# CVPR23/Depth-guided-Texture-Diffusion-for-Image-Semantic-Segmentation

Measured on AMD Instinct MI355X. Metric: training images/sec (512x512 RGB-D, bs=8 per GPU; fwd+loss+bwd+allreduce+AdamW), higher is better.
Workload: dtype bf16; 1 GPU; config/sod.yml model `cod` (pvt_v2_b2 + ConvNeXt-B texture diffuser + Hitnet decoder), 512x512 RGB+depth, batch 8/GPU, random init, DropPath active; mode=train, global_batch=8, parallelism=dp1, hip_graph=True, graph_mode=single

## Files before the change

depth-guided-texture-diffusion-for-image-semantic-segmentation_amd/csrc/attn_bwd.hip:

```cpp
#include "common.h"

namespace {

constexpr float LOG2E = 1.4426950408889634f;
constexpr int SLICE = 256;

template <typename T>
__global__ __launch_bounds__(256) void attn_delta_kernel(const T* __restrict__ o, const T* __restrict__ dout,
                                                         float* __restrict__ delta, int B, int N, int heads) {
  typedef typename Vec16<T>::type VT;
  constexpr int V = Vec16<T>::N, LPR = 64 / V;
  const int64_t total = (int64_t)B * N * heads;
  const int64_t gid = ((int64_t)blockIdx.x * 256 + threadIdx.x);
  const int64_t item = gid / LPR;
  const int sub = (int)(gid % LPR);
  float s = 0.f;
  int64_t bn = 0; int hd = 0;
  if (item < total) {
    bn = item / heads; hd = (int)(item % heads);
    const size_t off = ((size_t)bn * heads + hd) * 64 + sub * V;
    VT a = *reinterpret_cast<const VT*>(o + off);
    VT g = *reinterpret_cast<const VT*>(dout + off);
#pragma unroll
    for (int j = 0; j < V; ++j) s += (float)a[j] * (float)g[j];
  }
  s = group_sum(s, LPR);
  if (item < total && sub == 0) {
    const int64_t b = bn / N, n = bn % N;
    delta[((size_t)b * heads + hd) * N + n] = s;
  }
}

template <typename T>
struct DkdvSmem {
  static constexpr int QS = 72;
  T q[2][32][QS];
  T g[2][32][QS];
  float lse2[2][32];
  float dl[2][32];
};

constexpr int KGROUP = 128;
constexpr int64_t DKDV_MAX_WGS = 1024;
constexpr int64_t DKDV_SLAB_BYTES = DKDV_MAX_WGS * 65536;

template <typename T>
__global__ __launch_bounds__(256, 2) void sra_bwd_dkdv_bf16(const T* __restrict__ q, const T* __restrict__ kv,
                                                            const T* __restrict__ dout, const float* __restrict__ lse,
                                                            const float* __restrict__ delta, float* __restrict__ dkv,
                                                            int N, int Nkv, int heads, int kgroups, float scale, int qch,
                                                            int64_t slab_stride) {
  typedef T bf16_t;
  typedef typename Vec16<T>::type bf16x8;
  __shared__ __attribute__((aligned(16))) DkdvSmem<T> sm;
  constexpr int QS = DkdvSmem<T>::QS;
  const int C = heads * 64;
  const int b = blockIdx.z, hd = blockIdx.y / kgroups, kg = blockIdx.y % kgroups;
  const int tid = threadIdx.x, wave = tid >> 6, lane = tid & 63, r = lane & 31, h = lane >> 5;
  const float sl2 = scale * LOG2E;
  const bf16_t* kvb = kv + (size_t)b * Nkv * 2 * C + hd * 64;
  const size_t sbase = ((size_t)b * heads + hd) * N;
  const int qt_begin = blockIdx.x * qch;
  const int qt_end = min(qt_begin + qch, (N + 31) / 32);
  const int ktile0 = kg * KGROUP + wave * 32;
  const bool wave_active = ktile0 < Nkv;
  const int key = ktile0 + r;
  const bool kok = key < Nkv;

  auto stage_load = [&](int q0, bf16x8 (&v)[2], float& sv) {
#pragma unroll
    for (int k = 0; k < 2; ++k) {
      const int row = tid >> 3, ch = tid & 7;
      if (q0 + row < N) v[k] = *reinterpret_cast<const bf16x8*>((k ? dout : q) + ((size_t)b * N + q0 + row) * C + hd * 64 + ch * 8);
      else
#pragma unroll
        for (int j = 0; j < 8; ++j) v[k][j] = (bf16_t)0.f;
    }
    if (tid < 64) {
      const int row = tid & 31;
      const bool ok = (q0 + row) < N;
      sv = tid < 32 ? (ok ? lse[sbase + q0 + row] * LOG2E : INFINITY) : (ok ? delta[sbase + q0 + row] : 0.f);
    }
  };
  auto stage_store = [&](int buf, const bf16x8 (&v)[2], float sv) {
    const int row = tid >> 3, ch = tid & 7;
    *reinterpret_cast<bf16x8*>(&sm.q[buf][row][ch * 8]) = v[0];
    *reinterpret_cast<bf16x8*>(&sm.g[buf][row][ch * 8]) = v[1];
    if (tid < 32) sm.lse2[buf][tid] = sv;
    else if (tid < 64) sm.dl[buf][tid - 32] = sv;
  };

  bf16x8 kf[4], vf[4];
  {
    const bf16_t* kp = kvb + (size_t)key * 2 * C + 8 * h;
#pragma unroll
    for (int s = 0; s < 4; ++s) {
      if (kok) { kf[s] = *reinterpret_cast<const bf16x8*>(kp + 16 * s); vf[s] = *reinterpret_cast<const bf16x8*>(kp + C + 16 * s); }
      else
#pragma unroll
        for (int j = 0; j < 8; ++j) { kf[s][j] = (bf16_t)0.f; vf[s][j] = (bf16_t)0.f; }
    }
  }
  f32x16 dk[2], dv[2];
#pragma unroll
  for (int i = 0; i < 16; ++i) { dk[0][i] = dk[1][i] = dv[0][i] = dv[1][i] = 0.f; }

  bf16x8 st[2];
  float sv = 0.f;
  stage_load(qt_begin * 32, st, sv);
  stage_store(0, st, sv);
  __syncthreads();
  int cur = 0;
#pragma unroll 1
  for (int qt = qt_begin; qt < qt_end; ++qt) {
    const bool more = (qt + 1) < qt_end;
    if (more) stage_load((qt + 1) * 32, st, sv);
    if (wave_active) {
      f32x16 sA, pA;
#pragma unroll
      for (int i = 0; i < 16; ++i) { sA[i] = 0.f; pA[i] = 0.f; }
#pragma unroll
      for (int s = 0; s < 4; ++s) {
        const bf16x8 qf = *reinterpret_cast<const bf16x8*>(&sm.q[cur][r][16 * s + 8 * h]);
        const bf16x8 gf = *reinterpret_cast<const bf16x8*>(&sm.g[cur][r][16 * s + 8 * h]);
        sA = mfma16(qf, kf[s], sA);
        pA = mfma16(gf, vf[s], pA);
      }
#pragma unroll
      for (int i = 0; i < 16; ++i) {
        const int qi = mfma_row(i, h);
        const float p = kok ? __builtin_amdgcn_exp2f(fmaf(sA[i], sl2, -sm.lse2[cur][qi])) : 0.f;
        sA[i] = p;
        pA[i] = p * (pA[i] - sm.dl[cur][qi]) * scale;
      }
#pragma unroll
      for (int s2 = 0; s2 < 2; ++s2) {
        bf16x8 pf, df;
#pragma unroll
        for (int j = 0; j < 8; ++j) { pf[j] = (bf16_t)sA[8 * s2 + j]; df[j] = (bf16_t)pA[8 * s2 + j]; }
#pragma unroll
        for (int nb = 0; nb < 2; ++nb) {
          const bf16x8 gb = lds_tr_frag(&sm.g[cur][0][0], QS, 16 * s2, nb * 32, lane);
          const bf16x8 qb = lds_tr_frag(&sm.q[cur][0][0], QS, 16 * s2, nb * 32, lane);
          dv[nb] = mfma16(pf, gb, dv[nb]);
          dk[nb] = mfma16(df, qb, dk[nb]);
        }
      }
    }
    if (more) stage_store(cur ^ 1, st, sv);
    __syncthreads();
    cur ^= 1;
  }
  if (wave_active) {
#pragma unroll
    for (int nb = 0; nb < 2; ++nb)
#pragma unroll
      for (int i = 0; i < 16; ++i) {
        const int kk = ktile0 + mfma_row(i, h);
        if (kk < Nkv) {
          float* p = dkv + (size_t)blockIdx.x * slab_stride + ((size_t)b * Nkv + kk) * 2 * C + hd * 64 + nb * 32 + r;
          p[0] = dk[nb][i];
          p[C] = dv[nb][i];
        }
      }
  }
}

__global__ __launch_bounds__(256) void dkdv_reduce_kernel(const float* __restrict__ slab, float* __restrict__ dkv, int64_t n4, int chunks,
                                                          int64_t stride4) {
  const f32x4* s4 = reinterpret_cast<const f32x4*>(slab);
  f32x4* o4 = reinterpret_cast<f32x4*>(dkv);
  for (int64_t i = (int64_t)blockIdx.x * 256 + threadIdx.x; i < n4; i += (int64_t)gridDim.x * 256) {
    f32x4 acc = s4[i];
    for (int c = 1; c < chunks; ++c) {
      const f32x4 v = s4[i + (int64_t)c * stride4];
      acc[0] += v[0]; acc[1] += v[1]; acc[2] += v[2]; acc[3] += v[3];
    }
    o4[i] = acc;
  }
// ... 364 lines not shown
```

depth-guided-texture-diffusion-for-image-semantic-segmentation_amd/csrc/common.h:

```cpp
#pragma once
#include <hip/hip_runtime.h>
#include <stdint.h>
#include <stdio.h>
#include <stdlib.h>
#include "../../include/dgtd.h"

typedef __bf16 bf16_t;
typedef __bf16 bf16x8 __attribute__((ext_vector_type(8)));
typedef __bf16 bf16x4 __attribute__((ext_vector_type(4)));
typedef _Float16 f16_t;
typedef _Float16 f16x8 __attribute__((ext_vector_type(8)));
typedef _Float16 f16x4 __attribute__((ext_vector_type(4)));
typedef float f32x4 __attribute__((ext_vector_type(4)));
typedef float f32x16 __attribute__((ext_vector_type(16)));

void dgtd_set_error(const char* fmt, ...);
#define DGTD_FAIL(code, ...) do { dgtd_set_error(__VA_ARGS__); return (code); } while (0)
#define DGTD_REQUIRE(cond, ...) do { if (!(cond)) DGTD_FAIL(2, __VA_ARGS__); } while (0)
#define DGTD_CHECK_LAUNCH(name) do { hipError_t e_ = hipGetLastError(); \
    if (e_ != hipSuccess) DGTD_FAIL(3, "%s: launch failed: %s", name, hipGetErrorString(e_)); } while (0)

struct DgtdProfScope {
  bool on;
  hipEvent_t a, b;
  hipStream_t st;
  int bound;
  double amount;
  char key[112];
  DgtdProfScope(hipStream_t st, int bound, double amount, const char* fmt, ...) __attribute__((format(printf, 5, 6)));
  ~DgtdProfScope();
};
#define DGTD_PROF(st, bound, amount, ...) DgtdProfScope dgtd_prof_scope_((hipStream_t)(st), (bound), (double)(amount), __VA_ARGS__)
enum { DGTD_HBM = 0, DGTD_MFMA = 1 };
static inline int dgtd_esize(dgtd_dtype dt) { return (dt == DGTD_BF16 || dt == DGTD_F16) ? 2 : (dt == DGTD_F64 ? 8 : 4); }

template <typename T> __device__ __forceinline__ float to_f(T v) { return (float)v; }
template <typename T> __device__ __forceinline__ T from_f(float v) { return (T)v; }

template <typename T> struct Vec16;
template <> struct Vec16<float> { static constexpr int N = 4; typedef f32x4 type; };
template <> struct Vec16<bf16_t> { static constexpr int N = 8; typedef bf16x8 type; };
template <> struct Vec16<f16_t> { static constexpr int N = 8; typedef f16x8 type; };
template <typename T> struct Vec8;
template <> struct Vec8<bf16_t> { typedef bf16x4 type; };
template <> struct Vec8<f16_t> { typedef f16x4 type; };
template <typename T> struct Vec2;
template <> struct Vec2<float> { typedef float type __attribute__((ext_vector_type(2))); };
template <> struct Vec2<bf16_t> { typedef bf16_t type __attribute__((ext_vector_type(2))); };
template <> struct Vec2<f16_t> { typedef f16_t type __attribute__((ext_vector_type(2))); };

__device__ __forceinline__ f32x16 mfma16(bf16x8 a, bf16x8 b, f32x16 c) { return __builtin_amdgcn_mfma_f32_32x32x16_bf16(a, b, c, 0, 0, 0); }
__device__ __forceinline__ f32x16 mfma16(f16x8 a, f16x8 b, f32x16 c) { return __builtin_amdgcn_mfma_f32_32x32x16_f16(a, b, c, 0, 0, 0); }

#define DGTD_IS_HALF(dt) ((dt) == DGTD_BF16 || (dt) == DGTD_F16)
#define DGTD_DISPATCH(dt, STMT) do { if ((dt) == DGTD_BF16) { typedef bf16_t T_; STMT; } else if ((dt) == DGTD_F16) { typedef f16_t T_; STMT; } \
                                     else { typedef float T_; STMT; } } while (0)
#define DGTD_DISPATCH_HALF(dt, STMT) do { if ((dt) == DGTD_F16) { typedef f16_t T_; STMT; } else { typedef bf16_t T_; STMT; } } while (0)
#define DGTD_DISPATCH_K37(K, STMT) do { if ((K) == 7) { constexpr int K_ = 7; STMT; } else { constexpr int K_ = 3; STMT; } } while (0)

static inline long env_int(const char* name, long dflt) { const char* e = getenv(name); return e ? atol(e) : dflt; }

__device__ __forceinline__ float wave_sum(float v) {
#pragma unroll
  for (int o = 32; o > 0; o >>= 1) v += __shfl_xor(v, o, 64);
  return v;
}
__device__ __forceinline__ float wave_max(float v) {
#pragma unroll
  for (int o = 32; o > 0; o >>= 1) v = fmaxf(v, __shfl_xor(v, o, 64));
  return v;
}
__device__ __forceinline__ float group_sum(float v, int g) {
  for (int o = g >> 1; o > 0; o >>= 1) v += __shfl_xor(v, o, 64);
  return v;
}

__device__ __forceinline__ constexpr int mfma_row(int reg, int h) { return (reg & 3) + 8 * (reg >> 2) + 4 * h; }

typedef short s16x4 __attribute__((ext_vector_type(4)));
template <typename T>
__device__ __forceinline__ typename Vec16<T>::type lds_tr_frag(const T* base, int stride, int row0, int col0, int lane) {
  const int i = lane & 15, g1 = (lane >> 4) & 1, h = lane >> 5;
  const T* p = base + (row0 + 4 * h + (i >> 2)) * stride + col0 + 16 * g1 + 4 * (i & 3);
  typedef s16x4 __attribute__((address_space(3))) * lds_ptr;
  typedef typename Vec8<T>::type V4;
  s16x4 lo = __builtin_amdgcn_ds_read_tr16_b64_v4i16((lds_ptr)p);
  s16x4 hi = __builtin_amdgcn_ds_read_tr16_b64_v4i16((lds_ptr)(p + 8 * stride));
  V4 l4 = __builtin_bit_cast(V4, lo), h4 = __builtin_bit_cast(V4, hi);
  typename Vec16<T>::type f;
#pragma unroll
  for (int j = 0; j < 4; ++j) { f[j] = l4[j]; f[4 + j] = h4[j]; }
  return f;
}

__device__ __forceinline__ float gelu_phi(float x, float* pdf) {
  const float a = fabsf(x) * 0.70710678118654752f;
  const float t = __builtin_amdgcn_rcpf(fmaf(0.3275911f, a, 1.f));
  const float q = t * fmaf(t, fmaf(t, fmaf(t, fmaf(t, 1.061405429f, -1.453152027f), 1.421413741f), -0.284496736f), 0.254829592f);
  const float e = __builtin_amdgcn_exp2f(-a * a * 1.4426950408889634f);
  const float hc = 0.5f * q * e;
  *pdf = 0.3989422804014327f * e;
  return x >= 0.f ? 1.f - hc : hc;
}
__device__ __forceinline__ float gelu_fast(float x) { float pdf; return x * gelu_phi(x, &pdf); }
__device__ __forceinline__ float gelu_grad_fast(float x) { float pdf; const float phi = gelu_phi(x, &pdf); return fmaf(x, pdf, phi); }

static inline int64_t cdiv(int64_t a, int64_t b) { return (a + b - 1) / b; }

int dgtd_multi_reduce_impl(const dgtd_reduce_entry* entries, int n, hipStream_t st);
```

depth-guided-texture-diffusion-for-image-semantic-segmentation_amd/csrc/dwconv_tiled.hip:

```cpp
#include "common.h"

namespace {

constexpr int TY = 4, TXW = 16, TXS = 8;

template <typename T, int K>
__device__ __forceinline__ void stage_tile(T* __restrict__ tile, const T* __restrict__ x, int b, int y0, int x0, int cb, int H, int W,
                                           int C, int tid) {
  typedef typename Vec16<T>::type VT;
  constexpr int V = Vec16<T>::N, P = K / 2, RW = TXW + K - 1, RH = TY + K - 1, CPP = 128 / V;
  constexpr int TOTAL = RH * RW * CPP, NCH = (TOTAL + 255) / 256;
  VT v[NCH];
#pragma unroll
  for (int k = 0; k < NCH; ++k) {
    const int i = tid + k * 256;
    const int ch = i % CPP, pos = i / CPP, xx = pos % RW, yy = pos / RW;
    const int gy = y0 + yy - P, gx = x0 + xx - P;
    if (i < TOTAL && gy >= 0 && gy < H && gx >= 0 && gx < W) v[k] = *reinterpret_cast<const VT*>(x + (((size_t)b * H + gy) * W + gx) * C + cb * 128 + ch * V);
    else
#pragma unroll
      for (int j = 0; j < V; ++j) v[k][j] = (T)0.f;
  }
#pragma unroll
  for (int k = 0; k < NCH; ++k) {
    const int i = tid + k * 256;
    if (i < TOTAL) *reinterpret_cast<VT*>(tile + (size_t)i * V) = v[k];
  }
}

template <typename T, int K, int MODE>
__global__ __launch_bounds__(256) void dwconv_tiled_fwd_kernel(const T* __restrict__ x, const float* __restrict__ wt,
                                                               const float* __restrict__ bias, const T* __restrict__ aux,
                                                               T* __restrict__ y, int B, int H, int W, int C) {
  typedef typename Vec2<T>::type PT;
  constexpr int P = K / 2, RW = TXW + K - 1;
  extern __shared__ __attribute__((aligned(16))) char smem[];
  T* tile = reinterpret_cast<T*>(smem);
  const int tid = threadIdx.x, lane = tid & 63, wave = tid >> 6;
  const int ncb = C / 128, txn = (W + TXW - 1) / TXW, tyn = (H + TY - 1) / TY;
  const int nb = gridDim.x, xcd = blockIdx.x & 7, qn = nb >> 3, rn = nb & 7;
  int t = (xcd < rn ? xcd * (qn + 1) : rn * (qn + 1) + (xcd - rn) * qn) + (blockIdx.x >> 3);
  const int cb = t % ncb; t /= ncb;
  const int ty = t % tyn; t /= tyn;
  const int tx = t % txn;
  const int b = t / txn;
  const int y0 = ty * TY, x0 = tx * TXW, c0 = cb * 128 + lane * 2;
  stage_tile<T, K>(tile, x, b, y0, x0, cb, H, W, C, tid);
  typedef float f2 __attribute__((ext_vector_type(2)));
  f2 w[K * K];
#pragma unroll
  for (int i = 0; i < K * K; ++i) { w[i][0] = wt[(size_t)i * C + c0]; w[i][1] = wt[(size_t)i * C + c0 + 1]; }
  f2 bv;
  bv[0] = bias ? bias[c0] : 0.f; bv[1] = bias ? bias[c0 + 1] : 0.f;
  __syncthreads();
  const int oy = y0 + wave;
  if (oy >= H) return;
#pragma unroll 1
  for (int s = 0; s < TXW / TXS; ++s) {
    const int sx = s * TXS;
    if (x0 + sx >= W) break;
    f2 acc[TXS];
#pragma unroll
    for (int i = 0; i < TXS; ++i) acc[i] = bv;
#pragma unroll
    for (int ky = 0; ky < K; ++ky) {
      f2 in[TXS + K - 1];
      const T* row = tile + ((size_t)(wave + ky) * RW + sx) * 128 + lane * 2;
#pragma unroll
      for (int i = 0; i < TXS + K - 1; ++i) {
        PT v = *reinterpret_cast<const PT*>(row + (size_t)i * 128);
        in[i][0] = (float)v[0]; in[i][1] = (float)v[1];
      }
#pragma unroll
      for (int kx = 0; kx < K; ++kx)
#pragma unroll
        for (int i = 0; i < TXS; ++i) acc[i] = __builtin_elementwise_fma(in[i + kx], w[ky * K + kx], acc[i]);
    }
#pragma unroll
    for (int i = 0; i < TXS; ++i) {
      const int ox = x0 + sx + i;
      if (ox < W) {
        const size_t o = (((size_t)b * H + oy) * W + ox) * C + c0;
        PT r;
        if (MODE == 2) {
          PT g = *reinterpret_cast<const PT*>(aux + o);
          r[0] = (T)((float)g[0] * gelu_grad_fast(acc[i][0])); r[1] = (T)((float)g[1] * gelu_grad_fast(acc[i][1]));
        } else if (MODE == 1) {
          r[0] = (T)gelu_fast(acc[i][0]); r[1] = (T)gelu_fast(acc[i][1]);
        } else if (MODE == 3) {
          PT g = *reinterpret_cast<const PT*>(aux + o);
          r[0] = (T)(acc[i][0] + (float)g[0]); r[1] = (T)(acc[i][1] + (float)g[1]);
        } else {
          r[0] = (T)acc[i][0]; r[1] = (T)acc[i][1];
        }
        *reinterpret_cast<PT*>(y + o) = r;
      }
    }
  }
}

template <typename T, int K> constexpr size_t fwd_lds() { return (size_t)(TY + K - 1) * (TXW + K - 1) * 128 * sizeof(T); }

}

template <typename T, int K>
static int tiled_fwd(const void* x, const float* wt, const float* bias, const void* aux, void* y, int B, int H, int W, int C, int mode,
                     hipStream_t s) {
  const int64_t tiles = (int64_t)B * cdiv(H, TY) * cdiv(W, TXW) * (C / 128);
  DGTD_REQUIRE(tiles < (1LL << 31), "dwconv_tiled_fwd: too many tiles");
  const size_t lds = fwd_lds<T, K>();
#define TILED(MODE) hipLaunchKernelGGL((dwconv_tiled_fwd_kernel<T, K, MODE>), dim3((unsigned)tiles), dim3(256), lds, s, (const T*)x, wt, bias, (const T*)aux, (T*)y, B, H, W, C)
  if (mode == 0) TILED(0); else if (mode == 1) TILED(1); else if (mode == 2) TILED(2); else TILED(3);
#undef TILED
  DGTD_CHECK_LAUNCH("dwconv_tiled_fwd");
  return 0;
}

int dgtd_dwconv_tiled_fwd(const void* x, const float* wt, const float* bias, const void* aux, void* y, int B, int H, int W, int C, int K,
                          int mode, dgtd_dtype dt, hipStream_t s) {
  DGTD_REQUIRE(K == 7, "dwconv_tiled_fwd: K=%d (the tiled kernel serves 7x7 only)", K);
  DGTD_DISPATCH(dt, return (tiled_fwd<T_, 7>(x, wt, bias, aux, y, B, H, W, C, mode, s)));
}
```

depth-guided-texture-diffusion-for-image-semantic-segmentation_amd/csrc/layernorm.hip:

```cpp
#include "common.h"

namespace {

constexpr int LN_MAX_NPL = 4;
constexpr int LN_BWD_MAX_GRID = 1024;

template <typename T>
struct RowRegs {
  static constexpr int V = Vec16<T>::N;
  float v[LN_MAX_NPL][V];
};

template <typename T, int NPL>
__device__ __forceinline__ void load_row(const T* __restrict__ p, int cpr, int gl, int G, float (&v)[NPL][Vec16<T>::N]) {
  typedef typename Vec16<T>::type VT;
  constexpr int V = Vec16<T>::N;
#pragma unroll
  for (int i = 0; i < NPL; ++i) {
    int c = gl + i * G;
    if (c < cpr) {
      VT t = *reinterpret_cast<const VT*>(p + (size_t)c * V);
#pragma unroll
      for (int j = 0; j < V; ++j) v[i][j] = (float)t[j];
    } else {
#pragma unroll
      for (int j = 0; j < V; ++j) v[i][j] = 0.f;
    }
  }
}

template <typename T, int NPL>
__global__ __launch_bounds__(256) void ln_fwd_kernel(const T* __restrict__ x, const float* __restrict__ gamma,
                                                     const float* __restrict__ beta, T* __restrict__ y,
                                                     float* __restrict__ mean, float* __restrict__ rstd,
                                                     int64_t rows, int C, float eps, int G) {
  typedef typename Vec16<T>::type VT;
  constexpr int V = Vec16<T>::N;
  const int cpr = C / V;
  const int lane = threadIdx.x & 63, wave = threadIdx.x >> 6;
  const int gl = lane & (G - 1), gi = lane / G, rpw = 64 / G;
  const int64_t rows_per_block = (int64_t)rpw * 4;
  const float invC = 1.f / (float)C;
  float gm[NPL][V], bt[NPL][V];
#pragma unroll
  for (int i = 0; i < NPL; ++i) {
    int c = gl + i * G;
#pragma unroll
    for (int j = 0; j < V; ++j) {
      gm[i][j] = (c < cpr) ? gamma[c * V + j] : 0.f;
      bt[i][j] = (c < cpr) ? beta[c * V + j] : 0.f;
    }
  }
  constexpr int U = (NPL <= 2) ? 4 : 2;
  for (int64_t r0 = (int64_t)blockIdx.x * rows_per_block * U; r0 < rows; r0 += (int64_t)gridDim.x * rows_per_block * U) {
    float v[U][NPL][V];
    bool ok[U];
#pragma unroll
    for (int u = 0; u < U; ++u) {
      const int64_t row = r0 + (int64_t)u * rows_per_block + wave * rpw + gi;
      ok[u] = row < rows;
      if (ok[u]) load_row<T, NPL>(x + row * C, cpr, gl, G, v[u]);
      else {
#pragma unroll
        for (int i = 0; i < NPL; ++i)
#pragma unroll
          for (int j = 0; j < V; ++j) v[u][i][j] = 0.f;
      }
    }
#pragma unroll
    for (int u = 0; u < U; ++u) {
      const int64_t row = r0 + (int64_t)u * rows_per_block + wave * rpw + gi;
      float s = 0.f;
#pragma unroll
      for (int i = 0; i < NPL; ++i)
#pragma unroll
        for (int j = 0; j < V; ++j) s += v[u][i][j];
      const float mu = group_sum(s, G) * invC;
      float q = 0.f;
#pragma unroll
      for (int i = 0; i < NPL; ++i) {
        bool in = (gl + i * G) < cpr;
#pragma unroll
        for (int j = 0; j < V; ++j) { float d = in ? v[u][i][j] - mu : 0.f; q += d * d; }
      }
      const float rs = rsqrtf(group_sum(q, G) * invC + eps);
      if (ok[u]) {
#pragma unroll
        for (int i = 0; i < NPL; ++i) {
          int c = gl + i * G;
          if (c < cpr) {
            VT o;
#pragma unroll
            for (int j = 0; j < V; ++j) o[j] = (T)((v[u][i][j] - mu) * rs * gm[i][j] + bt[i][j]);
            *reinterpret_cast<VT*>(y + row * C + (size_t)c * V) = o;
          }
        }
        if (gl == 0) { mean[row] = mu; rstd[row] = rs; }
      }
    }
  }
}

template <typename T, int NPL>
__global__ __launch_bounds__(256) void ln_bwd_kernel(const T* __restrict__ dy, const T* __restrict__ x,
                                                     const float* __restrict__ gamma, const float* __restrict__ mean,
                                                     const float* __restrict__ rstd, const T* __restrict__ dres, T* __restrict__ dx,
                                                     float* __restrict__ ws, int64_t rows, int C, int G) {
  typedef typename Vec16<T>::type VT;
  constexpr int V = Vec16<T>::N;
  extern __shared__ float red[];
  const int cpr = C / V;
  const int lane = threadIdx.x & 63, wave = threadIdx.x >> 6;
  const int gl = lane & (G - 1), gi = lane / G, rpw = 64 / G;
  const int64_t rows_per_block = (int64_t)rpw * 4;
  const float invC = 1.f / (float)C;
  float gm[NPL][V], dg[NPL][V], db[NPL][V];
#pragma unroll
  for (int i = 0; i < NPL; ++i) {
    int c = gl + i * G;
#pragma unroll
    for (int j = 0; j < V; ++j) { gm[i][j] = (c < cpr) ? gamma[c * V + j] : 0.f; dg[i][j] = 0.f; db[i][j] = 0.f; }
  }
  constexpr int U = (NPL <= 2) ? 4 : 2;
  for (int64_t r0 = (int64_t)blockIdx.x * rows_per_block * U; r0 < rows; r0 += (int64_t)gridDim.x * rows_per_block * U) {
    float xv[U][NPL][V], gv[U][NPL][V], mu[U], rs[U];
    bool ok[U];
#pragma unroll
    for (int u = 0; u < U; ++u) {
      const int64_t row = r0 + (int64_t)u * rows_per_block + wave * rpw + gi;
      ok[u] = row < rows;
      if (ok[u]) {
        load_row<T, NPL>(x + row * C, cpr, gl, G, xv[u]);
        load_row<T, NPL>(dy + row * C, cpr, gl, G, gv[u]);
        mu[u] = mean[row]; rs[u] = rstd[row];
      } else {
        mu[u] = 0.f; rs[u] = 0.f;
#pragma unroll
        for (int i = 0; i < NPL; ++i)
#pragma unroll
          for (int j = 0; j < V; ++j) { xv[u][i][j] = 0.f; gv[u][i][j] = 0.f; }
      }
    }
#pragma unroll
    for (int u = 0; u < U; ++u) {
      float a = 0.f, b = 0.f;
#pragma unroll
      for (int i = 0; i < NPL; ++i) {
        bool in = (gl + i * G) < cpr;
#pragma unroll
        for (int j = 0; j < V; ++j) {
          float xh = in ? (xv[u][i][j] - mu[u]) * rs[u] : 0.f;
          float g = gv[u][i][j];
          dg[i][j] += g * xh;
          db[i][j] += g;
          g *= gm[i][j];
          a += g; b += g * xh;
          xv[u][i][j] = xh; gv[u][i][j] = g;
        }
      }
      a = group_sum(a, G) * invC;
      b = group_sum(b, G) * invC;
      if (ok[u]) {
        const int64_t row = r0 + (int64_t)u * rows_per_block + wave * rpw + gi;
#pragma unroll
        for (int i = 0; i < NPL; ++i) {
          int c = gl + i * G;
          if (c < cpr) {
            VT o, r;
            if (dres) r = *reinterpret_cast<const VT*>(dres + row * C + (size_t)c * V);
#pragma unroll
            for (int j = 0; j < V; ++j) o[j] = (T)(rs[u] * (gv[u][i][j] - a - xv[u][i][j] * b) + (dres ? (float)r[j] : 0.f));
            *reinterpret_cast<VT*>(dx + row * C + (size_t)c * V) = o;
          }
        }
      }
    }
  }
#pragma unroll
  for (int i = 0; i < NPL; ++i)
#pragma unroll
    for (int j = 0; j < V; ++j)
      for (int o = G; o < 64; o <<= 1) { dg[i][j] += __shfl_xor(dg[i][j], o, 64); db[i][j] += __shfl_xor(db[i][j], o, 64); }
  if (gi == 0) {
#pragma unroll
    for (int i = 0; i < NPL; ++i) {
      int c = gl + i * G;
      if (c < cpr)
#pragma unroll
        for (int j = 0; j < V; ++j) { red[(wave * 2 + 0) * C + c * V + j] = dg[i][j]; red[(wave * 2 + 1) * C + c * V + j] = db[i][j]; }
    }
  }
  __syncthreads();
  for (int c = threadIdx.x; c < 2 * C; c += 256) {
    int which = c / C, col = c % C;
    float s = 0.f;
#pragma unroll
    for (int w = 0; w < 4; ++w) s += red[(w * 2 + which) * C + col];
    ws[((size_t)blockIdx.x * 2 + which) * C + col] = s;
  }
}

struct LnGeom { int G, npl; int64_t rows_per_block; };
template <typename T> LnGeom ln_geom(int C) {
  int cpr = C / Vec16<T>::N;
  int G = 1;
  while (G < cpr && G < 64) G <<= 1;
  LnGeom g; g.G = G; g.npl = (cpr + G - 1) / G; g.rows_per_block = (64 / G) * 4;
  return g;
}

template <typename T>
int ln_fwd_launch(const void* x, const float* gamma, const float* beta, void* y, float* mean, float* rstd,
                  int64_t rows, int C, float eps, hipStream_t s) {
  DGTD_REQUIRE(C % Vec16<T>::N == 0, "layernorm: C=%d must be a multiple of %d", C, Vec16<T>::N);
  LnGeom g = ln_geom<T>(C);
  DGTD_REQUIRE(g.npl <= LN_MAX_NPL, "layernorm: C=%d too large", C);
  if (rows == 0) return 0;
  const int U = g.npl <= 2 ? 4 : 2;
  int grid = (int)std::min<int64_t>(cdiv(rows, g.rows_per_block * U), 256 * 8);
#define LN_FWD(NPL) hipLaunchKernelGGL((ln_fwd_kernel<T, NPL>), dim3(grid), dim3(256), 0, s, (const T*)x, gamma, beta, (T*)y, mean, rstd, rows, C, eps, g.G)
  switch (g.npl) { case 1: LN_FWD(1); break; case 2: LN_FWD(2); break; case 3: LN_FWD(3); break; default: LN_FWD(4); }
#undef LN_FWD
  DGTD_CHECK_LAUNCH("layernorm_fwd");
  return 0;
}

template <typename T>
int ln_bwd_launch(const void* dy, const void* x, const float* gamma, const float* mean, const float* rstd, void* dx,
                  float* dgamma, float* dbeta, void* ws, int64_t rows, int C, hipStream_t s, const void* dres = nullptr, int* nblocks = nullptr) {
  DGTD_REQUIRE(C % Vec16<T>::N == 0, "layernorm: C=%d must be a multiple of %d", C, Vec16<T>::N);
  LnGeom g = ln_geom<T>(C);
  DGTD_REQUIRE(g.npl <= LN_MAX_NPL, "layernorm: C=%d too large", C);
  DGTD_REQUIRE(rows > 0, "layernorm_bwd: rows must be > 0");
  int grid = (int)std::min<int64_t>(cdiv(rows, g.rows_per_block * 4), LN_BWD_MAX_GRID);
  size_t lds = (size_t)4 * 2 * C * sizeof(float);
#define LN_BWD(NPL) hipLaunchKernelGGL((ln_bwd_kernel<T, NPL>), dim3(grid), dim3(256), lds, s, (const T*)dy, (const T*)x, gamma, mean, rstd, (const T*)dres, (T*)dx, (float*)ws, rows, C, g.G)
  switch (g.npl) { case 1: LN_BWD(1); break; case 2: LN_BWD(2); break; case 3: LN_BWD(3); break; default: LN_BWD(4); }
#undef LN_BWD
  DGTD_CHECK_LAUNCH("layernorm_bwd");
  if (nblocks) { *nblocks = grid; return 0; }
  const dgtd_reduce_entry e{(const float*)ws, grid, 2 * C, dgamma, C, dbeta, DGTD_F32, 0, 0, nullptr};
  return dgtd_multi_reduce_impl(&e, 1, s);
}

}

extern "C" int dgtd_layernorm_fwd(const void* x, const float* gamma, const float* beta, void* y, float* mean, float* rstd,
                                  int64_t rows, int C, float eps, dgtd_dtype dt, dgtd_stream s) {
  DGTD_PROF(s, DGTD_HBM, 2.0 * dgtd_esize(dt) * rows * C, "dgtd_layernorm_fwd[rows=%lld,C=%d]", (long long)rows, C);
  DGTD_REQUIRE(DGTD_IS_HALF(dt) || dt == DGTD_F32, "layernorm_fwd: bad dtype %d", (int)dt);
  DGTD_DISPATCH(dt, return ln_fwd_launch<T_>(x, gamma, beta, y, mean, rstd, rows, C, eps, (hipStream_t)s));
}

extern "C" int dgtd_layernorm_bwd_add(const void* dy, const void* x, const float* gamma, const float* mean, const float* rstd,
                                      const void* dx_add, void* dx, float* dgamma, float* dbeta, void* workspace, int64_t rows, int C,
                                      dgtd_dtype dt, dgtd_stream s) {
  DGTD_PROF(s, DGTD_HBM, (dx_add ? 4.0 : 3.0) * dgtd_esize(dt) * rows * C, "dgtd_layernorm_bwd[rows=%lld,C=%d]", (long long)rows, C);
  DGTD_REQUIRE(DGTD_IS_HALF(dt) || dt == DGTD_F32, "layernorm_bwd_add: bad dtype %d", (int)dt);
  DGTD_DISPATCH(dt, return ln_bwd_launch<T_>(dy, x, gamma, mean, rstd, dx, dgamma, dbeta, workspace, rows, C, (hipStream_t)s, dx_add));
}

extern "C" int dgtd_layernorm_bwd_partial(const void* dy, const void* x, const float* gamma, const float* mean, const float* rstd,
                                          const void* dx_add, void* dx, void* workspace, int64_t rows, int C, dgtd_dtype dt, int* nblocks,
                                          dgtd_stream s) {
  DGTD_REQUIRE(nblocks, "layernorm_bwd_partial: nblocks is NULL");
  DGTD_PROF(s, DGTD_HBM, (dx_add ? 4.0 : 3.0) * dgtd_esize(dt) * rows * C, "dgtd_layernorm_bwd[rows=%lld,C=%d]", (long long)rows, C);
  DGTD_REQUIRE(DGTD_IS_HALF(dt) || dt == DGTD_F32, "layernorm_bwd_partial: bad dtype %d", (int)dt);
  DGTD_DISPATCH(dt, return ln_bwd_launch<T_>(dy, x, gamma, mean, rstd, dx, nullptr, nullptr, workspace, rows, C, (hipStream_t)s, dx_add, nblocks));
}

extern "C" int64_t dgtd_layernorm_bwd_workspace(int C) { return (int64_t)LN_BWD_MAX_GRID * 2 * C * sizeof(float); }

extern "C" int dgtd_layernorm_bwd(const void* dy, const void* x, const float* gamma, const float* mean, const float* rstd,
                                  void* dx, float* dgamma, float* dbeta, void* workspace, int64_t rows, int C,
                                  dgtd_dtype dt, dgtd_stream s) {
  DGTD_PROF(s, DGTD_HBM, 3.0 * dgtd_esize(dt) * rows * C, "dgtd_layernorm_bwd[rows=%lld,C=%d]", (long long)rows, C);
  DGTD_REQUIRE(DGTD_IS_HALF(dt) || dt == DGTD_F32, "layernorm_bwd: bad dtype %d", (int)dt);
  DGTD_DISPATCH(dt, return ln_bwd_launch<T_>(dy, x, gamma, mean, rstd, dx, dgamma, dbeta, workspace, rows, C, (hipStream_t)s));
}
```

Measured before the change: 275.5 images/s.

## Use DPP/permlane reductions, compile-time LN group size, and prefetch in dwconv

Replaces shuffle-based warp reductions with DPP and permlane swap intrinsics and makes the group size a template parameter. LayerNorm forward and backward now batch the group reductions across rows, clamp row indices so loads are unconditional, and are dispatched per (NPL, G). The depthwise conv tile stage splits its loads from its LDS stores, with clamped addresses instead of branches, and prefetches the aux (gradient or residual) inputs before the barrier. The aim is less cross-lane shuffle latency and better memory-level parallelism, at the cost of more template instantiations and more registers in use.

```diff
diff --git a/depth-guided-texture-diffusion-for-image-semantic-segmentation_amd/csrc/attn_bwd.hip b/depth-guided-texture-diffusion-for-image-semantic-segmentation_amd/csrc/attn_bwd.hip
--- a/depth-guided-texture-diffusion-for-image-semantic-segmentation_amd/csrc/attn_bwd.hip
+++ b/depth-guided-texture-diffusion-for-image-semantic-segmentation_amd/csrc/attn_bwd.hip
@@ -24,7 +24,7 @@
 #pragma unroll
     for (int j = 0; j < V; ++j) s += (float)a[j] * (float)g[j];
   }
-  s = group_sum(s, LPR);
+  s = group_sum<LPR>(s);
   if (item < total && sub == 0) {
     const int64_t b = bn / N, n = bn % N;
     delta[((size_t)b * heads + hd) * N + n] = s;
diff --git a/depth-guided-texture-diffusion-for-image-semantic-segmentation_amd/csrc/common.h b/depth-guided-texture-diffusion-for-image-semantic-segmentation_amd/csrc/common.h
--- a/depth-guided-texture-diffusion-for-image-semantic-segmentation_amd/csrc/common.h
+++ b/depth-guided-texture-diffusion-for-image-semantic-segmentation_amd/csrc/common.h
@@ -60,20 +60,51 @@
 
 static inline long env_int(const char* name, long dflt) { const char* e = getenv(name); return e ? atol(e) : dflt; }
 
-__device__ __forceinline__ float wave_sum(float v) {
+struct LaneAdd { __device__ __forceinline__ float operator()(float a, float b) const { return a + b; } };
+struct LaneMax { __device__ __forceinline__ float operator()(float a, float b) const { return fmaxf(a, b); } };
+
+template <int CTRL, int BANK_MASK>
+__device__ __forceinline__ float dpp_move(float old, float v) {
+  return __builtin_bit_cast(float, __builtin_amdgcn_update_dpp(__builtin_bit_cast(int, old), __builtin_bit_cast(int, v), CTRL, 0xF, BANK_MASK, false));
+}
+template <int O, bool INV8 = false, typename Op>
+__device__ __forceinline__ float lane_xor_combine(float v, Op op) {
+  static_assert(O == 1 || O == 2 || O == 4 || O == 8 || O == 16 || O == 32, "lane_xor_combine: O must be a power of two below 64");
+  if constexpr (O == 1) return op(v, dpp_move<0xB1, 0xF>(v, v));
+  else if constexpr (O == 2) return op(v, dpp_move<0x4E, 0xF>(v, v));
+  else if constexpr (O == 4 && INV8) return op(v, dpp_move<0x124, 0xF>(v, v));
+  else if constexpr (O == 4) return op(v, dpp_move<0x114, 0xA>(dpp_move<0x104, 0x5>(v, v), v));
+  else if constexpr (O == 8) return op(v, dpp_move<0x128, 0xF>(v, v));
+  else {
+    const unsigned u = __builtin_bit_cast(unsigned, v);
+    const auto r = (O == 16) ? __builtin_amdgcn_permlane16_swap(u, u, false, false) : __builtin_amdgcn_permlane32_swap(u, u, false, false);
+    return op(__builtin_bit_cast(float, (unsigned)r[0]), __builtin_bit_cast(float, (unsigned)r[1]));
+  }
+}
+template <int G, int N, typename Op>
+__device__ __forceinline__ void group_reduce(float (&v)[N], Op op) {
+  static_assert(G == 1 || G == 2 || G == 4 || G == 8 || G == 16 || G == 32 || G == 64, "group_reduce: G must be a power of two <= 64");
 #pragma unroll
-  for (int o = 32; o > 0; o >>= 1) v += __shfl_xor(v, o, 64);
-  return v;
+  for (int n = 0; n < N; ++n) if constexpr (G >= 64) v[n] = lane_xor_combine<32>(v[n], op);
+#pragma unroll
+  for (int n = 0; n < N; ++n) if constexpr (G >= 32) v[n] = lane_xor_combine<16>(v[n], op);
+#pragma unroll
+  for (int n = 0; n < N; ++n) if constexpr (G >= 16) v[n] = lane_xor_combine<8>(v[n], op);
+#pragma unroll
+  for (int n = 0; n < N; ++n) if constexpr (G >= 8) v[n] = lane_xor_combine<4, (G >= 16)>(v[n], op);
+#pragma unroll
+  for (int n = 0; n < N; ++n) if constexpr (G >= 4) v[n] = lane_xor_combine<2>(v[n], op);
+#pragma unroll
+  for (int n = 0; n < N; ++n) if constexpr (G >= 2) v[n] = lane_xor_combine<1>(v[n], op);
 }
-__device__ __forceinline__ float wave_max(float v) {
+template <int O, int N> __device__ __forceinline__ void lane_xor_add(float (&v)[N]) {
 #pragma unroll
-  for (int o = 32; o > 0; o >>= 1) v = fmaxf(v, __shfl_xor(v, o, 64));
-  return v;
+  for (int n = 0; n < N; ++n) v[n] = lane_xor_combine<O>(v[n], LaneAdd());
 }
-__device__ __forceinline__ float group_sum(float v, int g) {
-  for (int o = g >> 1; o > 0; o >>= 1) v += __shfl_xor(v, o, 64);
-  return v;
-}
+template <int G, int N> __device__ __forceinline__ void group_sum(float (&v)[N]) { group_reduce<G>(v, LaneAdd()); }
+template <int G> __device__ __forceinline__ float group_sum(float v) { float a[1] = {v}; group_reduce<G>(a, LaneAdd()); return a[0]; }
+__device__ __forceinline__ float wave_sum(float v) { return group_sum<64>(v); }
+__device__ __forceinline__ float wave_max(float v) { float a[1] = {v}; group_reduce<64>(a, LaneMax()); return a[0]; }
 
 __device__ __forceinline__ constexpr int mfma_row(int reg, int h) { return (reg & 3) + 8 * (reg >> 2) + 4 * h; }
 
diff --git a/depth-guided-texture-diffusion-for-image-semantic-segmentation_amd/csrc/dwconv_tiled.hip b/depth-guided-texture-diffusion-for-image-semantic-segmentation_amd/csrc/dwconv_tiled.hip
--- a/depth-guided-texture-diffusion-for-image-semantic-segmentation_amd/csrc/dwconv_tiled.hip
+++ b/depth-guided-texture-diffusion-for-image-semantic-segmentation_amd/csrc/dwconv_tiled.hip
@@ -5,27 +5,40 @@
 constexpr int TY = 4, TXW = 16, TXS = 8;
 
 template <typename T, int K>
-__device__ __forceinline__ void stage_tile(T* __restrict__ tile, const T* __restrict__ x, int b, int y0, int x0, int cb, int H, int W,
-                                           int C, int tid) {
+struct TileStage {
   typedef typename Vec16<T>::type VT;
-  constexpr int V = Vec16<T>::N, P = K / 2, RW = TXW + K - 1, RH = TY + K - 1, CPP = 128 / V;
-  constexpr int TOTAL = RH * RW * CPP, NCH = (TOTAL + 255) / 256;
+  static constexpr int V = Vec16<T>::N, P = K / 2, RW = TXW + K - 1, RH = TY + K - 1, CPP = 128 / V;
+  static constexpr int TOTAL = RH * RW * CPP, NCH = (TOTAL + 255) / 256, SLOTS = NCH * 256;
   VT v[NCH];
+  bool ok[NCH];
+  __device__ __forceinline__ void load(const T* __restrict__ x, int b, int y0, int x0, int cb, int H, int W, int C, int tid) {
 #pragma unroll
-  for (int k = 0; k < NCH; ++k) {
-    const int i = tid + k * 256;
-    const int ch = i % CPP, pos = i / CPP, xx = pos % RW, yy = pos / RW;
-    const int gy = y0 + yy - P, gx = x0 + xx - P;
-    if (i < TOTAL && gy >= 0 && gy < H && gx >= 0 && gx < W) v[k] = *reinterpret_cast<const VT*>(x + (((size_t)b * H + gy) * W + gx) * C + cb * 128 + ch * V);
-    else
+    for (int k = 0; k < NCH; ++k) {
+      const int i = tid + k * 256;
+      const int ch = i % CPP, pos = i / CPP, xx = pos % RW, yy = pos / RW;
+      const int gy = y0 + yy - P, gx = x0 + xx - P;
+      ok[k] = i < TOTAL && gy >= 0 && gy < H && gx >= 0 && gx < W;
+      const int cy = min(max(gy, 0), H - 1), cx = min(max(gx, 0), W - 1);
+      v[k] = *reinterpret_cast<const VT*>(x + (((size_t)b * H + cy) * W + cx) * C + cb * 128 + ch * V);
+    }
+  }
+  __device__ __forceinline__ void store(T* __restrict__ tile, int tid) const {
 #pragma unroll
-      for (int j = 0; j < V; ++j) v[k][j] = (T)0.f;
+    for (int k = 0; k < NCH; ++k) {
+      const int i = tid + k * 256;
+      VT o;
+#pragma unroll
+      for (int j = 0; j < V; ++j) o[j] = ok[k] ? v[k][j] : (T)0.f;
+      *reinterpret_cast<VT*>(tile + (size_t)i * V) = o;
+    }
   }
-#pragma unroll
-  for (int k = 0; k < NCH; ++k) {
-    const int i = tid + k * 256;
-    if (i < TOTAL) *reinterpret_cast<VT*>(tile + (size_t)i * V) = v[k];
-  }
+};
+
+template <typename P>
+__device__ __forceinline__ void pin_here(P& v) {
+  static_assert(sizeof(P) == 4 || sizeof(P) == 8, "pin_here: one or two registers");
+  if constexpr (sizeof(P) == 4) { unsigned u = __builtin_bit_cast(unsigned, v); asm volatile("" : "+v"(u)); v = __builtin_bit_cast(P, u); }
+  else { unsigned long long u = __builtin_bit_cast(unsigned long long, v); asm volatile("" : "+v"(u)); v = __builtin_bit_cast(P, u); }
 }
 
 template <typename T, int K, int MODE>
@@ -45,16 +58,30 @@
   const int tx = t % txn;
   const int b = t / txn;
   const int y0 = ty * TY, x0 = tx * TXW, c0 = cb * 128 + lane * 2;
-  stage_tile<T, K>(tile, x, b, y0, x0, cb, H, W, C, tid);
+  TileStage<T, K> st;
+  st.load(x, b, y0, x0, cb, H, W, C, tid);
   typedef float f2 __attribute__((ext_vector_type(2)));
   f2 w[K * K];
 #pragma unroll
   for (int i = 0; i < K * K; ++i) { w[i][0] = wt[(size_t)i * C + c0]; w[i][1] = wt[(size_t)i * C + c0 + 1]; }
+  const float* bp = bias ? bias : wt;
+  const float b0 = bp[c0], b1 = bp[c0 + 1];
   f2 bv;
-  bv[0] = bias ? bias[c0] : 0.f; bv[1] = bias ? bias[c0 + 1] : 0.f;
+  bv[0] = bias ? b0 : 0.f; bv[1] = bias ? b1 : 0.f;
+  const int oy = y0 + wave;
+  static_assert(TXW == 2 * TXS, "the aux prefetch holds two strips");
+  PT ax[TXS], ax_next[TXS];
+  if (MODE >= 2) {
+    const size_t arow = ((size_t)b * H + min(oy, H - 1)) * W;
+#pragma unroll
+    for (int i = 0; i < TXS; ++i) {
+      ax[i] = *reinterpret_cast<const PT*>(aux + (arow + min(x0 + i, W - 1)) * C + c0);
+      ax_next[i] = *reinterpret_cast<const PT*>(aux + (arow + min(x0 + TXS + i, W - 1)) * C + c0);
+    }
+  }
+  __builtin_amdgcn_sched_barrier(0);
+  st.store(tile, tid);
   __syncthreads();
-  const int oy = y0 + wave;
-  if (oy >= H) return;
 #pragma unroll 1
   for (int s = 0; s < TXW / TXS; ++s) {
     const int sx = s * TXS;
@@ -77,18 +104,20 @@
         for (int i = 0; i < TXS; ++i) acc[i] = __builtin_elementwise_fma(in[i + kx], w[ky * K + kx], acc[i]);
     }
 #pragma unroll
+    for (int i = 0; i < TXS; ++i) { pin_here(acc[i]); if (MODE >= 2) pin_here(ax[i]); }
+#pragma unroll
     for (int i = 0; i < TXS; ++i) {
       const int ox = x0 + sx + i;
-      if (ox < W) {
+      if (ox < W && oy < H) {
         const size_t o = (((size_t)b * H + oy) * W + ox) * C + c0;
         PT r;
         if (MODE == 2) {
-          PT g = *reinterpret_cast<const PT*>(aux + o);
+          const PT g = ax[i];
           r[0] = (T)((float)g[0] * gelu_grad_fast(acc[i][0])); r[1] = (T)((float)g[1] * gelu_grad_fast(acc[i][1]));
         } else if (MODE == 1) {
           r[0] = (T)gelu_fast(acc[i][0]); r[1] = (T)gelu_fast(acc[i][1]);
         } else if (MODE == 3) {
-          PT g = *reinterpret_cast<const PT*>(aux + o);
+          const PT g = ax[i];
           r[0] = (T)(acc[i][0] + (float)g[0]); r[1] = (T)(acc[i][1] + (float)g[1]);
         } else {
           r[0] = (T)acc[i][0]; r[1] = (T)acc[i][1];
@@ -96,10 +125,14 @@
         *reinterpret_cast<PT*>(y + o) = r;
       }
     }
+    if (MODE >= 2) {
+#pragma unroll
+      for (int i = 0; i < TXS; ++i) ax[i] = ax_next[i];
+    }
   }
 }
 
-template <typename T, int K> constexpr size_t fwd_lds() { return (size_t)(TY + K - 1) * (TXW + K - 1) * 128 * sizeof(T); }
+template <typename T, int K> constexpr size_t fwd_lds() { return (size_t)TileStage<T, K>::SLOTS * 16; }
 
 }
 
diff --git a/depth-guided-texture-diffusion-for-image-semantic-segmentation_amd/csrc/layernorm.hip b/depth-guided-texture-diffusion-for-image-semantic-segmentation_amd/csrc/layernorm.hip
--- a/depth-guided-texture-diffusion-for-image-semantic-segmentation_amd/csrc/layernorm.hip
+++ b/depth-guided-texture-diffusion-for-image-semantic-segmentation_amd/csrc/layernorm.hip
@@ -4,190 +4,203 @@
 
 constexpr int LN_MAX_NPL = 4;
 constexpr int LN_BWD_MAX_GRID = 1024;
-
-template <typename T>
-struct RowRegs {
+constexpr int ln_rows_in_flight(int npl) { return npl <= 2 ? 4 : 2; }
+
+typedef float f32x4_a4 __attribute__((ext_vector_type(4), aligned(4)));
+
+template <typename T, int NPL, int G>
+struct LnLane {
   static constexpr int V = Vec16<T>::N;
-  float v[LN_MAX_NPL][V];
+  bool in[NPL];
+  int off[NPL];
+  __device__ __forceinline__ LnLane(int gl, int cpr) {
+#pragma unroll
+    for (int i = 0; i < NPL; ++i) { const int c = gl + i * G; in[i] = c < cpr; off[i] = (in[i] ? c : cpr - 1) * V; }
+  }
+  __device__ __forceinline__ void load_param(const float* __restrict__ p, float (&o)[NPL][V]) const {
+    f32x4 t[NPL][V / 4];
+#pragma unroll
+    for (int i = 0; i < NPL; ++i)
+#pragma unroll
+      for (int k = 0; k < V / 4; ++k) t[i][k] = *reinterpret_cast<const f32x4_a4*>(p + off[i] + 4 * k);
+#pragma unroll
+    for (int i = 0; i < NPL; ++i)
+#pragma unroll
+      for (int j = 0; j < V; ++j) o[i][j] = in[i] ? t[i][j / 4][j % 4] : 0.f;
+  }
 };
 
-template <typename T, int NPL>
-__device__ __forceinline__ void load_row(const T* __restrict__ p, int cpr, int gl, int G, float (&v)[NPL][Vec16<T>::N]) {
-  typedef typename Vec16<T>::type VT;
-  constexpr int V = Vec16<T>::N;
-#pragma unroll
-  for (int i = 0; i < NPL; ++i) {
-    int c = gl + i * G;
-    if (c < cpr) {
-      VT t = *reinterpret_cast<const VT*>(p + (size_t)c * V);
-#pragma unroll
-      for (int j = 0; j < V; ++j) v[i][j] = (float)t[j];
-    } else {
-#pragma unroll
-      for (int j = 0; j < V; ++j) v[i][j] = 0.f;
-    }
-  }
-}
-
-template <typename T, int NPL>
+template <typename T, int NPL, int G>
 __global__ __launch_bounds__(256) void ln_fwd_kernel(const T* __restrict__ x, const float* __restrict__ gamma,
                                                      const float* __restrict__ beta, T* __restrict__ y,
                                                      float* __restrict__ mean, float* __restrict__ rstd,
-                                                     int64_t rows, int C, float eps, int G) {
+                                                     int64_t rows, int C, float eps) {
   typedef typename Vec16<T>::type VT;
-  constexpr int V = Vec16<T>::N;
-  const int cpr = C / V;
+  constexpr int V = Vec16<T>::N, U = ln_rows_in_flight(NPL), RPW = 64 / G, RPB = RPW * 4;
   const int lane = threadIdx.x & 63, wave = threadIdx.x >> 6;
-  const int gl = lane & (G - 1), gi = lane / G, rpw = 64 / G;
-  const int64_t rows_per_block = (int64_t)rpw * 4;
+  const int gl = lane & (G - 1), gi = lane / G;
   const float invC = 1.f / (float)C;
+  const LnLane<T, NPL, G> ll(gl, C / V);
   float gm[NPL][V], bt[NPL][V];
-#pragma unroll
-  for (int i = 0; i < NPL; ++i) {
-    int c = gl + i * G;
-#pragma unroll
-    for (int j = 0; j < V; ++j) {
-      gm[i][j] = (c < cpr) ? gamma[c * V + j] : 0.f;
-      bt[i][j] = (c < cpr) ? beta[c * V + j] : 0.f;
-    }
-  }
-  constexpr int U = (NPL <= 2) ? 4 : 2;
-  for (int64_t r0 = (int64_t)blockIdx.x * rows_per_block * U; r0 < rows; r0 += (int64_t)gridDim.x * rows_per_block * U) {
-    float v[U][NPL][V];
-    bool ok[U];
-#pragma unroll
-    for (int u = 0; u < U; ++u) {
-      const int64_t row = r0 + (int64_t)u * rows_per_block + wave * rpw + gi;
-      ok[u] = row < rows;
-      if (ok[u]) load_row<T, NPL>(x + row * C, cpr, gl, G, v[u]);
-      else {
-#pragma unroll
-        for (int i = 0; i < NPL; ++i)
-#pragma unroll
-          for (int j = 0; j < V; ++j) v[u][i][j] = 0.f;
-      }
-    }
-#pragma unroll
-    for (int u = 0; u < U; ++u) {
-      const int64_t row = r0 + (int64_t)u * rows_per_block + wave * rpw + gi;
-      float s = 0.f;
-#pragma unroll
-      for (int i = 0; i < NPL; ++i)
-#pragma unroll
-        for (int j = 0; j < V; ++j) s += v[u][i][j];
-      const float mu = group_sum(s, G) * invC;
-      float q = 0.f;
-#pragma unroll
-      for (int i = 0; i < NPL; ++i) {
-        bool in = (gl + i * G) < cpr;
-#pragma unroll
-        for (int j = 0; j < V; ++j) { float d = in ? v[u][i][j] - mu : 0.f; q += d * d; }
-      }
-      const float rs = rsqrtf(group_sum(q, G) * invC + eps);
-      if (ok[u]) {
-#pragma unroll
-        for (int i = 0; i < NPL; ++i) {
-          int c = gl + i * G;
-          if (c < cpr) {
-            VT o;
-#pragma unroll
-            for (int j = 0; j < V; ++j) o[j] = (T)((v[u][i][j] - mu) * rs * gm[i][j] + bt[i][j]);
-            *reinterpret_cast<VT*>(y + row * C + (size_t)c * V) = o;
-          }
-        }
-        if (gl == 0) { mean[row] = mu; rstd[row] = rs; }
-      }
-    }
-  }
-}
-
-template <typename T, int NPL>
+  ll.load_param(gamma, gm);
+  ll.load_param(beta, bt);
+  for (int64_t r0 = (int64_t)blockIdx.x * RPB * U; r0 < rows; r0 += (int64_t)gridDim.x * RPB * U) {
+    VT t[U][NPL];
+#pragma unroll
+    for (int u = 0; u < U; ++u) {
+      const int64_t rr = r0 + u * RPB + wave * RPW + gi, row = rr < rows ? rr : rows - 1;
+#pragma unroll
+      for (int i = 0; i < NPL; ++i) t[u][i] = *reinterpret_cast<const VT*>(x + row * C + ll.off[i]);
+    }
+    float v[U][NPL][V], s[U], q[U];
+#pragma unroll
+    for (int u = 0; u < U; ++u) {
+      s[u] = 0.f;
+#pragma unroll
+      for (int i = 0; i < NPL; ++i)
+#pragma unroll
+        for (int j = 0; j < V; ++j) { v[u][i][j] = ll.in[i] ? (float)t[u][i][j] : 0.f; s[u] += v[u][i][j]; }
+    }
+    group_sum<G>(s);
+#pragma unroll
+    for (int u = 0; u < U; ++u) {
+      s[u] *= invC;
+      q[u] = 0.f;
+#pragma unroll
+      for (int i = 0; i < NPL; ++i)
+#pragma unroll
+        for (int j = 0; j < V; ++j) { float d = ll.in[i] ? v[u][i][j] - s[u] : 0.f; q[u] = __builtin_fmaf(d, d, q[u]); }
+    }
+    group_sum<G>(q);
+    VT o[U][NPL];
+#pragma unroll
+    for (int u = 0; u < U; ++u) {
+      q[u] = rsqrtf(__builtin_fmaf(q[u], invC, eps));
+#pragma unroll
+      for (int i = 0; i < NPL; ++i)
+#pragma unroll
+        for (int j = 0; j < V; ++j) o[u][i][j] = (T)__builtin_fmaf((v[u][i][j] - s[u]) * q[u], gm[i][j], bt[i][j]);
+    }
+    auto store_row = [&](int u, int64_t row) {
+#pragma unroll
+      for (int i = 0; i < NPL; ++i)
+        if (ll.in[i]) *reinterpret_cast<VT*>(y + row * C + ll.off[i]) = o[u][i];
+      if (gl == 0) { mean[row] = s[u]; rstd[row] = q[u]; }
+    };
+    const int64_t first = r0 + wave * RPW + gi;
+    if (r0 + (int64_t)RPB * U <= rows) {
+#pragma unroll
+      for (int u = 0; u < U; ++u) store_row(u, first + u * RPB);
+    } else {
+#pragma unroll
+      for (int u = 0; u < U; ++u)
+        if (first + u * RPB < rows) store_row(u, first + u * RPB);
+    }
+  }
+}
+
+template <typename T, int NPL, int G>
 __global__ __launch_bounds__(256) void ln_bwd_kernel(const T* __restrict__ dy, const T* __restrict__ x,
                                                      const float* __restrict__ gamma, const float* __restrict__ mean,
                                                      const float* __restrict__ rstd, const T* __restrict__ dres, T* __restrict__ dx,
-                                                     float* __restrict__ ws, int64_t rows, int C, int G) {
+                                                     float* __restrict__ ws, int64_t rows, int C) {
   typedef typename Vec16<T>::type VT;
-  constexpr int V = Vec16<T>::N;
+  constexpr int V = Vec16<T>::N, U = ln_rows_in_flight(NPL), RPW = 64 / G, RPB = RPW * 4;
   extern __shared__ float red[];
-  const int cpr = C / V;
   const int lane = threadIdx.x & 63, wave = threadIdx.x >> 6;
-  const int gl = lane & (G - 1), gi = lane / G, rpw = 64 / G;
-  const int64_t rows_per_block = (int64_t)rpw * 4;
+  const int gl = lane & (G - 1), gi = lane / G;
   const float invC = 1.f / (float)C;
+  const LnLane<T, NPL, G> ll(gl, C / V);
   float gm[NPL][V], dg[NPL][V], db[NPL][V];
 #pragma unroll
-  for (int i = 0; i < NPL; ++i) {
-    int c = gl + i * G;
-#pragma unroll
-    for (int j = 0; j < V; ++j) { gm[i][j] = (c < cpr) ? gamma[c * V + j] : 0.f; dg[i][j] = 0.f; db[i][j] = 0.f; }
-  }
-  constexpr int U = (NPL <= 2) ? 4 : 2;
-  for (int64_t r0 = (int64_t)blockIdx.x * rows_per_block * U; r0 < rows; r0 += (int64_t)gridDim.x * rows_per_block * U) {
-    float xv[U][NPL][V], gv[U][NPL][V], mu[U], rs[U];
-    bool ok[U];
-#pragma unroll
-    for (int u = 0; u < U; ++u) {
-      const int64_t row = r0 + (int64_t)u * rows_per_block + wave * rpw + gi;
-      ok[u] = row < rows;
-      if (ok[u]) {
-        load_row<T, NPL>(x + row * C, cpr, gl, G, xv[u]);
-        load_row<T, NPL>(dy + row * C, cpr, gl, G, gv[u]);
-        mu[u] = mean[row]; rs[u] = rstd[row];
-      } else {
-        mu[u] = 0.f; rs[u] = 0.f;
-#pragma unroll
-        for (int i = 0; i < NPL; ++i)
-#pragma unroll
-          for (int j = 0; j < V; ++j) { xv[u][i][j] = 0.f; gv[u][i][j] = 0.f; }
+  for (int i = 0; i < NPL; ++i)
+#pragma unroll
+    for (int j = 0; j < V; ++j) { dg[i][j] = 0.f; db[i][j] = 0.f; }
+  ll.load_param(gamma, gm);
+  for (int64_t r0 = (int64_t)blockIdx.x * RPB * U; r0 < rows; r0 += (int64_t)gridDim.x * RPB * U) {
+    VT tx[U][NPL], tg[U][NPL], tr[U][NPL];
+    float mu[U], rs[U];
+#pragma unroll
+    for (int u = 0; u < U; ++u) {
+      const int64_t rr = r0 + u * RPB + wave * RPW + gi, row = rr < rows ? rr : rows - 1;
+#pragma unroll
+      for (int i = 0; i < NPL; ++i) {
+        tx[u][i] = *reinterpret_cast<const VT*>(x + row * C + ll.off[i]);
+        tg[u][i] = *reinterpret_cast<const VT*>(dy + row * C + ll.off[i]);
       }
-    }
-#pragma unroll
-    for (int u = 0; u < U; ++u) {
+      mu[u] = mean[row]; rs[u] = rstd[row];
+    }
+    if (dres) {
+#pragma unroll
+      for (int u = 0; u < U; ++u) {
+        const int64_t rr = r0 + u * RPB + wave * RPW + gi, row = rr < rows ? rr : rows - 1;
+#pragma unroll
+        for (int i = 0; i < NPL; ++i) tr[u][i] = *reinterpret_cast<const VT*>(dres + row * C + ll.off[i]);
+      }
+    }
+    const int64_t first = r0 + wave * RPW + gi;
+    const bool full = r0 + (int64_t)RPB * U <= rows;
+    float xv[U][NPL][V], gv[U][NPL][V], ab[2 * U];
+#pragma unroll
+    for (int u = 0; u < U; ++u) {
+      const bool ok = full || first + u * RPB < rows;
       float a = 0.f, b = 0.f;
 #pragma unroll
       for (int i = 0; i < NPL; ++i) {
-        bool in = (gl + i * G) < cpr;
+        const bool in = ll.in[i] && ok;
 #pragma unroll
         for (int j = 0; j < V; ++j) {
-          float xh = in ? (xv[u][i][j] - mu[u]) * rs[u] : 0.f;
-          float g = gv[u][i][j];
-          dg[i][j] += g * xh;
+          float xh = in ? ((float)tx[u][i][j] - mu[u]) * rs[u] : 0.f;
+          float g = in ? (float)tg[u][i][j] : 0.f;
+          dg[i][j] = __builtin_fmaf(g, xh, dg[i][j]);
           db[i][j] += g;
           g *= gm[i][j];
-          a += g; b += g * xh;
+          a += g; b = __builtin_fmaf(g, xh, b);
           xv[u][i][j] = xh; gv[u][i][j] = g;
         }
       }
-      a = group_sum(a, G) * invC;
-      b = group_sum(b, G) * invC;
-      if (ok[u]) {
-        const int64_t row = r0 + (int64_t)u * rows_per_block + wave * rpw + gi;
-#pragma unroll
-        for (int i = 0; i < NPL; ++i) {
-          int c = gl + i * G;
-          if (c < cpr) {
-            VT o, r;
-            if (dres) r = *reinterpret_cast<const VT*>(dres + row * C + (size_t)c * V);
-#pragma unroll
-            for (int j = 0; j < V; ++j) o[j] = (T)(rs[u] * (gv[u][i][j] - a - xv[u][i][j] * b) + (dres ? (float)r[j] : 0.f));
-            *reinterpret_cast<VT*>(dx + row * C + (size_t)c * V) = o;
-          }
-        }
-      }
-    }
-  }
-#pragma unroll
-  for (int i = 0; i < NPL; ++i)
-#pragma unroll
-    for (int j = 0; j < V; ++j)
-      for (int o = G; o < 64; o <<= 1) { dg[i][j] += __shfl_xor(dg[i][j], o, 64); db[i][j] += __shfl_xor(db[i][j], o, 64); }
+      ab[2 * u] = a; ab[2 * u + 1] = b;
+    }
+    group_sum<G>(ab);
+    VT o[U][NPL];
+#pragma unroll
+    for (int u = 0; u < U; ++u) {
+      const float a = ab[2 * u] * invC, b = ab[2 * u + 1] * invC;
+#pragma unroll
+      for (int i = 0; i < NPL; ++i)
+#pragma unroll
+        for (int j = 0; j < V; ++j)
+          o[u][i][j] = (T)__builtin_fmaf(rs[u], __builtin_fmaf(-xv[u][i][j], b, gv[u][i][j] - a), dres ? (float)tr[u][i][j] : 0.f);
+    }
+    auto store_row = [&](int u, int64_t row) {
+#pragma unroll
+      for (int i = 0; i < NPL; ++i)
+        if (ll.in[i]) *reinterpret_cast<VT*>(dx + row * C + ll.off[i]) = o[u][i];
+    };
+    if (full) {
+#pragma unroll
+      for (int u = 0; u < U; ++u) store_row(u, first + u * RPB);
+    } else {
+#pragma unroll
+      for (int u = 0; u < U; ++u)
+        if (first + u * RPB < rows) store_row(u, first + u * RPB);
+    }
+  }
+#pragma unroll
+  for (int i = 0; i < NPL; ++i) {
+    if constexpr (G <= 1)  { lane_xor_add<1>(dg[i]);  lane_xor_add<1>(db[i]); }
+    if constexpr (G <= 2)  { lane_xor_add<2>(dg[i]);  lane_xor_add<2>(db[i]); }
+    if constexpr (G <= 4)  { lane_xor_add<4>(dg[i]);  lane_xor_add<4>(db[i]); }
+    if constexpr (G <= 8)  { lane_xor_add<8>(dg[i]);  lane_xor_add<8>(db[i]); }
+    if constexpr (G <= 16) { lane_xor_add<16>(dg[i]); lane_xor_add<16>(db[i]); }
+    if constexpr (G <= 32) { lane_xor_add<32>(dg[i]); lane_xor_add<32>(db[i]); }
+  }
   if (gi == 0) {
 #pragma unroll
     for (int i = 0; i < NPL; ++i) {
-      int c = gl + i * G;
-      if (c < cpr)
-#pragma unroll
-        for (int j = 0; j < V; ++j) { red[(wave * 2 + 0) * C + c * V + j] = dg[i][j]; red[(wave * 2 + 1) * C + c * V + j] = db[i][j]; }
+      if (ll.in[i])
+#pragma unroll
+        for (int j = 0; j < V; ++j) { red[(wave * 2 + 0) * C + ll.off[i] + j] = dg[i][j]; red[(wave * 2 + 1) * C + ll.off[i] + j] = db[i][j]; }
     }
   }
   __syncthreads();
@@ -209,6 +222,15 @@
   return g;
 }
 
+#define LN_DISPATCH(g, STMT) do { \
+    if ((g).G == 64) { constexpr int G_ = 64; \
+      if ((g).npl == 1) { constexpr int NPL_ = 1; STMT; } else if ((g).npl == 2) { constexpr int NPL_ = 2; STMT; } \
+      else if ((g).npl == 3) { constexpr int NPL_ = 3; STMT; } else { constexpr int NPL_ = 4; STMT; } } \
+    else { constexpr int NPL_ = 1; \
+      if ((g).G == 32) { constexpr int G_ = 32; STMT; } else if ((g).G == 16) { constexpr int G_ = 16; STMT; } \
+      else if ((g).G == 8) { constexpr int G_ = 8; STMT; } else if ((g).G == 4) { constexpr int G_ = 4; STMT; } \
+      else if ((g).G == 2) { constexpr int G_ = 2; STMT; } else { constexpr int G_ = 1; STMT; } } } while (0)
+
 template <typename T>
 int ln_fwd_launch(const void* x, const float* gamma, const float* beta, void* y, float* mean, float* rstd,
                   int64_t rows, int C, float eps, hipStream_t s) {
@@ -216,11 +238,8 @@
   LnGeom g = ln_geom<T>(C);
   DGTD_REQUIRE(g.npl <= LN_MAX_NPL, "layernorm: C=%d too large", C);
   if (rows == 0) return 0;
-  const int U = g.npl <= 2 ? 4 : 2;
-  int grid = (int)std::min<int64_t>(cdiv(rows, g.rows_per_block * U), 256 * 8);
-#define LN_FWD(NPL) hipLaunchKernelGGL((ln_fwd_kernel<T, NPL>), dim3(grid), dim3(256), 0, s, (const T*)x, gamma, beta, (T*)y, mean, rstd, rows, C, eps, g.G)
-  switch (g.npl) { case 1: LN_FWD(1); break; case 2: LN_FWD(2); break; case 3: LN_FWD(3); break; default: LN_FWD(4); }
-#undef LN_FWD
+  int grid = (int)std::min<int64_t>(cdiv(rows, g.rows_per_block * ln_rows_in_flight(g.npl)), 256 * 8);
+  LN_DISPATCH(g, hipLaunchKernelGGL((ln_fwd_kernel<T, NPL_, G_>), dim3(grid), dim3(256), 0, s, (const T*)x, gamma, beta, (T*)y, mean, rstd, rows, C, eps));
   DGTD_CHECK_LAUNCH("layernorm_fwd");
   return 0;
 }
@@ -234,9 +253,7 @@
   DGTD_REQUIRE(rows > 0, "layernorm_bwd: rows must be > 0");
   int grid = (int)std::min<int64_t>(cdiv(rows, g.rows_per_block * 4), LN_BWD_MAX_GRID);
   size_t lds = (size_t)4 * 2 * C * sizeof(float);
-#define LN_BWD(NPL) hipLaunchKernelGGL((ln_bwd_kernel<T, NPL>), dim3(grid), dim3(256), lds, s, (const T*)dy, (const T*)x, gamma, mean, rstd, (const T*)dres, (T*)dx, (float*)ws, rows, C, g.G)
-  switch (g.npl) { case 1: LN_BWD(1); break; case 2: LN_BWD(2); break; case 3: LN_BWD(3); break; default: LN_BWD(4); }
-#undef LN_BWD
+  LN_DISPATCH(g, hipLaunchKernelGGL((ln_bwd_kernel<T, NPL_, G_>), dim3(grid), dim3(256), lds, s, (const T*)dy, (const T*)x, gamma, mean, rstd, (const T*)dres, (T*)dx, (float*)ws, rows, C));
   DGTD_CHECK_LAUNCH("layernorm_bwd");
   if (nblocks) { *nblocks = grid; return 0; }
   const dgtd_reduce_entry e{(const float*)ws, grid, 2 * C, dgamma, C, dbeta, DGTD_F32, 0, 0, nullptr};
```

New measurement: 287.1 images/s (median of 6 runs). 4.2% higher.
